# szpiech/garlic

Hardware: AMD Instinct MI355X
Metric: LOD-windows/sec (SNPs x inds / winsize) (higher is better)
Workload: dtype f64

## Files before the change

garlic_amd/csrc/garlic_hip.hip:

```cpp
#include "../../include/garlic_hip.h"
#include "lod_kernels.hpp"
#include "variant_kernels.hpp"
#include "ld_kernels.hpp"
#include "ld_multi_kernel.hpp"
#include "tgls_ring_kernel.hpp"
#include "tgls_wide_kernel.hpp"
#include "tgls_feed_kernel.hpp"
#include "tgls_feed_multi_kernel.hpp"
#include "wlod_strip_kernel.hpp"
#include "wlod_small_kernel.hpp"
#include "coverage_kernel.hpp"
#include "roh_segments_kernel.hpp"
#include "feed_kernel.hpp"
#include "wlod_feed_kernel.hpp"
#include "feed_sort_kernel.hpp"
#include "kde_kernels.hpp"
#include "../host/kde_select.hpp"
#include "bed_kernels.hpp"

#include <algorithm>
#include <chrono>
#include <functional>
#include <memory>
#include <mutex>
// ... 1981 lines not shown
    }
    for (int q = 0; q < 2; q++) {
        size_t blocks = 0;
        for (size_t k = (size_t)q; k < n_slabs; k += 2) blocks = std::max(blocks, (size_t)(slabs[k].b1 - slabs[k].b0));
        const size_t need = blocks * (size_t)rows * WAVE;
        if (need > p->d_slab[q].cap || (!need && p->d_slab[q].cap)) {
            HIP_TRY(hipStreamSynchronize(s));
            p->d_slab[q].release();
            if (need && (rc = p->d_slab[q].reserve(need))) return rc;
        }
    }
    const bool wide = p->gl_wide, wide_host = wide && tgls_terms_on_host(p);
    if (wide) {
        if ((rc = ensure_log10(p->ctx)) || (rc = ensure_dfreq(p)) || (rc = ensure_values16(p))) return rc;
        p->gl_terms_by = p->slab_terms_by = tgls_terms_on_host(p) ? 2 : 1;
    }
    HIP_TRY(hipEventRecord(p->ev_slab_begin, s));
    HIP_TRY(hipStreamWaitEvent(p->slab_stream, p->ev_slab_begin, 0));
    VariantArgs a{p->d_packed.p, nullptr, p->d_tabgl.p, p->d_codes.p, nullptr, nullptr, nullptr, nullptr, nullptr,
                  p->nind_pad, p->nwordrows, 0, 0, 0, (int32_t)p->gl_values.size(), 1, nullptr, 0};
    const size_t terms_lds = sizeof(double) * GL_TERMS_S * 4 * (size_t)a.ncodes;
    if (!wide && terms_lds > LDS_DEFAULT_MAX)
        HIP_TRY(hipFuncSetAttribute((const void *)gl_terms_slab_kernel, hipFuncAttributeMaxDynamicSharedMemorySize, (int)terms_lds));
    const unsigned terms_grid = (unsigned)((p->nloci + GL_TERMS_S - 1) / GL_TERMS_S + (GL_PAD_ROWS + GL_TERMS_S - 1) / GL_TERMS_S);
    for (size_t k = 0; k < n_slabs; k++) {
        const Plan::Slab &sl = slabs[k];
        const int q = (int)(k & 1);
        if (k >= 2) HIP_TRY(hipStreamWaitEvent(p->slab_stream, p->ev_slab_read[q], 0));
        if (wide_host) {
            if ((rc = build_wide_terms_on_host(p, sl.b0, sl.b1, scaled ? p->h_decay.data() : nullptr, p->d_slab[q].p, p->slab_stream, nullptr)))
                return rc;
        } else if (wide)
            launch_wide_terms(p, sl.b0, sl.b1, scaled ? p->d_decay.p : nullptr, p->d_slab[q].p, nullptr, p->slab_stream);
        else
        hipLaunchKernelGGL(gl_terms_slab_kernel, dim3(terms_grid), dim3(256), terms_lds, p->slab_stream, a, p->nloci, rows, sl.b0, sl.b1,
                           scaled ? p->d_decay.p : (const double *)nullptr, p->d_slab[q].p);
        HIP_TRY(hipGetLastError());
        HIP_TRY(hipEventRecord(p->ev_slab_built[q], p->slab_stream));
        HIP_TRY(hipStreamWaitEvent(s, p->ev_slab_built[q], 0));
        if ((rc = chains(k, (const double *)p->d_slab[q].p))) return rc;
        HIP_TRY(hipGetLastError());
        HIP_TRY(hipEventRecord(p->ev_slab_read[q], s));
    }
    return GARLIC_OK;
}

int tgls_workers(const garlic_ctx *ctx, size_t n_items)
{
    int workers = ctx->n_cu;
    if (const char *e = getenv("GARLIC_WORKERS")) workers = std::max(1, atoi(e));
    return std::min<int>(workers, (int)n_items);
}

int launch_tgls_slabs(garlic_panel *p, const LodCall &c, const LodForm &form, const Plan &plan, double *d_out)
{
    hipStream_t s = p->ctx->stream;
    const int64_t rows = GOFF + p->nloci + GPAD_BACK;
    const size_t n_slabs = plan.slabs.size();
    int rc;
    if (n_slabs) {
        if ((rc = p->d_slab_queues.reserve(2 * n_slabs))) return rc;
        HIP_TRY(hipMemsetAsync(p->d_slab_queues.p, 0, 2 * n_slabs * sizeof(int32_t), s));
        if (form.cov_bits) p->cov_written = true;
    }
    return for_each_tgls_slab(p, plan.slabs, form.slab_blocks, [&](size_t k, const double *terms) {
        const Plan::Slab &sl = plan.slabs[k];
        const int workers = tgls_workers(p->ctx, sl.n_items);
        if (form.family == Family::tgls_feed) {
            TglsFeedArgs t{terms, rows, p->d_items.p + sl.item0, p->d_chrs.p, d_out,
                           c.ind_begin, c.ind_count, c.W, (int32_t)sl.n_items, c.thin_step, sl.b0, p->d_slab_queues.p + 2 * k};
            hipLaunchKernelGGL(tgls_feed_kernel, dim3((unsigned)workers), dim3(TGF_THREADS), 0, s, t);
        } else {
            TglsArgs t{terms, rows, p->d_items.p + sl.item0, p->d_chrs.p, d_out,
                       c.ind_begin, c.ind_count, c.W, (int32_t)sl.n_items, sl.b0, p->d_slab_queues.p + 2 * k, p->cov_pending};
            hipLaunchKernelGGL(lod_chain_ring_kernel, dim3((unsigned)workers), dim3(TG_THREADS), 0, s, t);
        }
        return (int)GARLIC_OK;
    });
}

int launch_tgls(garlic_panel *p, const LodCall &c, const LodForm &form, const Plan &plan, int workers, double *d_out)
{
    hipStream_t s = p->ctx->stream;
    const int64_t rows = GOFF + p->nloci + GPAD_BACK;
    if (form.cov_bits && !form.writes_bits) return GARLIC_INTERNAL_NO_BITS;
    p->last_slab_blocks = p->last_n_slabs = 0;
    if (form.slab_blocks && (form.family == Family::tgls_feed || form.family == Family::tgls_ring))
        return launch_tgls_slabs(p, c, form, plan, d_out);
    if (form.family == Family::tgls_feed) {
        TglsFeedArgs t{p->d_glterms.p, rows, p->d_items.p, p->d_chrs.p, d_out,
                       c.ind_begin, c.ind_count, c.W, (int32_t)plan.n_items, c.thin_step, 0, p->d_counter.p};
        hipLaunchKernelGGL(tgls_feed_kernel, dim3((unsigned)workers), dim3(TGF_THREADS), 0, s, t);
        return GARLIC_OK;
    }
    if (form.family == Family::tgls_ring) {
        TglsArgs t{p->d_glterms.p, rows, p->d_items.p, p->d_chrs.p, d_out,
                   c.ind_begin, c.ind_count, c.W, (int32_t)plan.n_items, 0, p->d_counter.p, p->cov_pending};
        if (form.cov_bits) p->cov_written = true;
        hipLaunchKernelGGL(lod_chain_ring_kernel, dim3((unsigned)workers), dim3(TG_THREADS), 0, s, t);
        return GARLIC_OK;
    }
    const VariantArgs a = variant_args(p, c, form, d_out);
    if (form.family == Family::tgls_terms)
        hipLaunchKernelGGL(lod_chain_terms_kernel, dim3((unsigned)plan.n_items), dim3(2 * WAVE), 0, s, a, (int)plan.n_items, rows, p->d_glterms.p);
    else
        hipLaunchKernelGGL(lod_chain_gl_kernel, dim3((unsigned)((plan.n_items + GL_WAVES - 1) / GL_WAVES)), dim3(GL_WAVES * WAVE), 0, s, a,
                           (int)plan.n_items);
    return GARLIC_OK;
}

int launch_generic_wlod(garlic_panel *p, const LodCall &c, const LodForm &form, const Plan &plan, double *d_out)
{
    const int ring = c.W + TILE;
    const size_t lds = sizeof(double) * ((size_t)ring * WAVE + ((c.W + 1) & ~1) + (size_t)WAVE * TPITCH);
    if (lds > 160 * 1024)
        return fail(GARLIC_ERR_INVALID, "wLOD with winsize %d: this build supports 2..240 and 16..4096", c.W);
    HIP_TRY(hipFuncSetAttribute(reinterpret_cast<const void *>(wlod_kernel), hipFuncAttributeMaxDynamicSharedMemorySize, (int)lds));
    hipLaunchKernelGGL(wlod_kernel, dim3((unsigned)plan.n_items), dim3(WAVE), lds, p->ctx->stream, variant_args(p, c, form, d_out), ring);
    return GARLIC_OK;
}

int launch_wlod_feed(garlic_panel *p, const LodCall &c, const LodForm &form, const Plan &plan, double *d_out, const WlodTerms &t,
                     int32_t fb0, int32_t n_fb)
{
    const int nquad = (n_fb + WFD_WAVES - 1) / WFD_WAVES;
    WlodFeedArgs a{p->d_packed.p, form.wlod_gl ? t.terms : p->d_wtab.p, p->d_skew.p + SKEW_FRONT, p->d_valid.p, p->d_chrs.p,
                   p->d_tiles.p, p->d_feed_blocks.p + fb0, d_out, p->nwordrows, GOFF + p->nloci + GPAD_BACK, c.ind_count, c.W, c.thin_step,
                   n_fb, nquad, (uint32_t)((int64_t)plan.n_tiles * nquad), t.blk0};
    if (!a.n_work) return GARLIC_OK;
    if (form.wlod_gl) hipLaunchKernelGGL(wlod_feed_kernel<true>, dim3(a.n_work), dim3(WFD_WAVES * WAVE), 0, p->ctx->stream, a);
    else hipLaunchKernelGGL(wlod_feed_kernel<false>, dim3(a.n_work), dim3(WFD_WAVES * WAVE), 0, p->ctx->stream, a);
    return GARLIC_OK;
}

int launch_wlod_slabs(garlic_panel *p, const LodCall &c, const LodForm &form, const Plan &plan, double *d_out)
{
    return for_each_tgls_slab(p, plan.slabs, form.slab_blocks, [&](size_t k, const double *terms) {
        const Plan::Slab &sl = plan.slabs[k];
        const WlodTerms t = wlod_terms_slab(c, sl, terms);
        if (form.family == Family::wlod_feed) return launch_wlod_feed(p, c, form, plan, d_out, t, sl.fb0, sl.n_fb);
        return launch_wlod(p, c, form, plan, d_out, t);
    }, true);
}

int enqueue_lod(garlic_panel *p, const LodCall &c, const LodForm &form, const Layout &L, Plan &plan, const LodWork *fresh,
                double *d_out, Family family)
{
    garlic_ctx *ctx = p->ctx;
    hipStream_t s = ctx->stream;
    int rc = GARLIC_OK;
    HIP_TRY(hipEventRecord(ctx->ev_begin, s));
    if (fresh && ((rc = p->d_chrs.put(fresh->chrs, s)) || (rc = p->d_items.put(fresh->items, s)) || (rc = p->d_fill.put(fresh->fill, s)) ||
// ... 1160 lines not shown
    return GARLIC_OK;
}
#define LD_COL_FNS(kernel) {kernel<1>, kernel<2>, kernel<3>, kernel<4>, kernel<5>}

static int ld_sum_table(garlic_panel *p, const LdForm &f, std::vector<LdSumChr> &chrs, unsigned *blocks)
{
    int64_t n = 0;
    for (int c = 0; c < p->nchr; c++) {
        const int64_t nstarts = p->chr_off[c + 1] - p->chr_off[c] - f.W + 1;
        if (nstarts < 1) continue;
        chrs.push_back(LdSumChr{p->chr_off[c], nstarts, n});
        n += (nstarts + f.sum_b - 1) / f.sum_b;
    }
    *blocks = (unsigned)n;
    return p->lds.sum_chrs.put(chrs, p->ctx->stream);
}

static int ld_sum_col(garlic_panel *p, const LdForm &f, double *ld, std::vector<LdSumChr> &chrs)
{
    int rc;
    unsigned nwork = 0;
    if ((rc = ld_sum_table(p, f, chrs, &nwork)) || (rc = reserve_skew(p, f.W, false))) return rc;
    if (chrs.empty()) return GARLIC_OK;
    decltype(&ld_sum_col_kernel<1>) const fns[] = LD_COL_FNS(ld_sum_col_kernel);
    return ld_launch_col(p, f, fns, 0, nwork, p->lds.fwd.p, p->lds.sum_chrs.p, (int)chrs.size(), f.W, f.sum_b, ld, p->d_skew.p + SKEW_FRONT);
}

static int ld_sum_two_tables(garlic_panel *p, const LdForm &f, const int32_t *pair, double *ld, std::vector<LdSumChr> &chrs)
{
    int rc;
    hipStream_t s = p->ctx->stream;
    const int32_t W = f.W;
    const size_t n = (size_t)p->nloci * W;
    if ((rc = p->lds.fwd.reserve(n)) || (rc = p->lds.bwd.reserve(n))) return rc;
    for (int c = 0; c < p->nchr; c++) {
        const int64_t lo = p->chr_off[c], hi = p->chr_off[c + 1];
        hipLaunchKernelGGL(ld_hr2_kernel<false>, dim3((unsigned)(hi - lo)), dim3(256), 0, s, pair, p->lds.hf.p, lo, hi, W, p->lds.fwd.p,
                           p->lds.bwd.p);
        if (f.sum == LdSum::plain && hi - lo >= W)
            hipLaunchKernelGGL(ld_sum_kernel, dim3((unsigned)(hi - lo - W + 1)), dim3(256), 0, s, p->lds.fwd.p, p->lds.bwd.p, lo, W, ld);
    }
    if (f.sum == LdSum::plain) return GARLIC_OK;
    unsigned blocks = 0;
    if ((rc = ld_sum_table(p, f, chrs, &blocks))) return rc;
    if (chrs.empty()) return GARLIC_OK;
    const size_t lds = sizeof(double) * 2 * (2 * (size_t)W - 1 + 128 + f.sum_threads);
    (void)hist_mark(p->ctx, false);
    hipLaunchKernelGGL(ld_sum_tiled_kernel, dim3(blocks), dim3(f.sum_threads), lds, s, p->lds.fwd.p, p->lds.bwd.p, p->lds.sum_chrs.p,
                       (int)chrs.size(), W, ld);
    (void)hist_mark(p->ctx, true);
    return GARLIC_OK;
}

static int ld_finish_run(garlic_panel *p, const LdForm &f, const int32_t *loc, const int32_t *pair, double *ld, bool have_table,
                         bool keep_sets)
{
    int rc;
    const bool col = f.sum == LdSum::col;
    if (ld && !col) HIP_TRY(hipMemsetAsync(ld, 0, sizeof(double) * (size_t)p->nloci * f.W, p->ctx->stream));
    if ((ld && col && (rc = ld_zero_short_rows(p, f.W, ld))) || (rc = ld_hf(p, f, loc))) return rc;
    std::vector<LdSumChr> chrs;
    switch (f.sum) {
    case LdSum::flat:
        (void)hist_mark(p->ctx, false);
        hipLaunchKernelGGL(ld_sum_flat_kernel, dim3((unsigned)(((size_t)p->nloci * f.W + 255) / 256)), dim3(256), 0, p->ctx->stream, pair,
                           p->lds.hf.p, p->d_chr_off.p, p->nchr, p->nloci, f.W, ld);
        (void)hist_mark(p->ctx, true);
        break;
    case LdSum::col:
        if (!have_table) rc = ld_build_table(p, f, pair);
        if (!rc) rc = ld_sum_col(p, f, ld, chrs);
        break;
    case LdSum::tiled:
    case LdSum::plain: rc = ld_sum_two_tables(p, f, pair, ld, chrs); break;
    }
    if (rc) return rc;
    HIP_TRY(hipGetLastError());
    return install_ld(p, f.W, ld, col, keep_sets);
}

static int ld_copy_out(double *dst, const double *src, size_t n, int32_t where)
{
    HIP_TRY(hipMemcpy(dst, src, sizeof(double) * n, where == GARLIC_HOST ? hipMemcpyDeviceToHost : hipMemcpyDeviceToDevice));
    return GARLIC_OK;
}

static int ld_finish_to(garlic_panel *p, const LdForm &f, const int32_t *loc, const int32_t *pair, bool have_table, double *ld_out,
                        bool host_out, bool keep_sets)
{
    int rc;
    const size_t n = (size_t)p->nloci * f.W;
    double *ld = host_out ? nullptr : ld_out;
    if (!ld && (ld_out || f.sum != LdSum::col)) {
        if ((rc = p->lds.ld.reserve(n))) return rc;
        ld = p->lds.ld.p;
    }
    if ((rc = ld_finish_run(p, f, loc, pair, ld, have_table, keep_sets))) return rc;
    return ld_out && ld != ld_out ? ld_copy_out(ld_out, ld, n, GARLIC_HOST) : GARLIC_OK;
}

int garlic_ld_finish(garlic_panel *p, int32_t winsize, int32_t phased, const int32_t *locus_counts,
                     const int32_t *pair_counts, double *ld_out, int32_t where)
{
    int rc;
    if ((rc = ld_check(p, winsize, phased))) return rc;
    if (!locus_counts || !pair_counts) return fail(GARLIC_ERR_INVALID, "count buffers are required");
    hipStream_t s = p->ctx->stream;
    if (where == GARLIC_HOST) {
        DevBuf<int32_t> &d_loc = p->lds.loc, &d_pair = p->lds.pair;
        const size_t npair = (size_t)p->nloci * winsize * 2;
        if ((rc = d_loc.reserve((size_t)p->nloci * 2)) || (rc = d_pair.reserve(npair))) return rc;
        HIP_TRY(hipMemcpyAsync(d_loc.p, locus_counts, sizeof(int32_t) * p->nloci * 2, hipMemcpyHostToDevice, s));
        HIP_TRY(hipMemcpyAsync(d_pair.p, pair_counts, sizeof(int32_t) * npair, hipMemcpyHostToDevice, s));
        locus_counts = d_loc.p; pair_counts = d_pair.p;
    }
    const LdForm f = ld_form(p, winsize, phased);
    ld_note_form(p, f, false);
    return ld_finish_to(p, f, locus_counts, pair_counts, false, ld_out, where == GARLIC_HOST, false);
}

static int ld_compute(garlic_panel *p, const LdForm &f, const std::vector<uint64_t> &sub, double *ld_out, bool host_out, bool keep_sets)
{
    int rc;
    DevBuf<int32_t> &d_loc = p->lds.loc, &d_pair = p->lds.pair;
    ld_note_form(p, f, f.fusable);
    if ((rc = d_loc.reserve((size_t)p->nloci * 2)) || (rc = d_pair.reserve(f.fusable ? 2 : (size_t)p->nloci * f.W * 2))) return rc;
    if ((rc = ld_counts_run(p, f, sub, d_loc.p, d_pair.p, f.fusable))) return rc;
    return ld_finish_to(p, f, d_loc.p, d_pair.p, f.fusable, ld_out, host_out, keep_sets);
}

int garlic_panel_compute_ld(garlic_panel *p, int32_t winsize, int32_t phased, const int32_t *sub_idx,
                            int32_t n_sub, double *ld_out, int32_t where)
{
    int rc;
    if ((rc = ld_check(p, winsize, phased))) return rc;
    std::vector<uint64_t> sub;
    if ((rc = ld_sub_bitmap(p, sub_idx, n_sub, sub))) return rc;
    return ld_compute(p, ld_form(p, winsize, phased), sub, ld_out, where != GARLIC_DEVICE, false);
}

struct LdMultiPlan {
    std::vector<int32_t> uniq;
    std::vector<std::vector<int32_t>> groups;
    size_t n_shared = 0;
    int32_t wtab = 0;
};
// ... 1107 lines not shown
            a_w0 = d_w0.p;
        }
        hipLaunchKernelGGL(roh_segments_from_mask_kernel, grid, dim3(256), 0, s, d_mask.p, bm.d_bchrs.p, d_brk.p, bm.d_wbase.p, p->nchr, p->nind, T,
                           d_segs.p, (long long)cap, d_count.p, a_w0);
        e = hipGetLastError();
        if (e == hipSuccess) e = hipMemcpyAsync(&found, d_count.p, sizeof found, hipMemcpyDeviceToHost, s);
        if (e == hipSuccess) e = hipStreamSynchronize(s);
        if (e != hipSuccess) return fail(GARLIC_ERR_HIP, "roh segments: %s", hipGetErrorString(e));
    }
    if (sink.n_out) *sink.n_out = (int64_t)found;
    if ((int64_t)found <= cap && found > 0) {
        e = hipMemcpyAsync(sink.segs, d_segs.p, sizeof(garlic_roh_segment) * found, hipMemcpyDeviceToHost, s);
        if (e == hipSuccess) e = hipStreamSynchronize(s);
        if (e != hipSuccess) return fail(GARLIC_ERR_HIP, "roh segments: %s", hipGetErrorString(e));
        std::sort(sink.segs, sink.segs + found, [](const garlic_roh_segment &x, const garlic_roh_segment &y) {
            return x.ind != y.ind ? x.ind < y.ind : x.chr != y.chr ? x.chr < y.chr : x.start < y.start;
        });
    }
    return GARLIC_OK;
}

static int coverage_unfused(garlic_panel *p, const CovSink &c)
{
    hipStream_t s = p->ctx->stream;
    const Layout L = make_layout(p, 32, p->nind);
    int rc;
    if ((rc = p->d_out.reserve(p->ctx, (size_t)L.total))) return rc;
    if (c.weighted) rc = garlic_wlod_windows(p, c.W, c.error, c.max_gap, c.use_gl, c.M, c.mu, 0, p->nind, 32, p->d_out.p, GARLIC_DEVICE);
    else rc = garlic_lod_windows(p, c.W, c.error, c.max_gap, c.use_gl, 0, p->nind, 32, p->d_out.p, GARLIC_DEVICE);
    if (rc) return rc;
    if (!c.segments) return garlic_roh_coverage(p, p->d_out.p, 32, p->nind, c.W, c.cutoff, c.inwin, c.inwin_pitch_align, c.where);
    const std::vector<ChrDev> schrs = chr_table(p, L);
    BitMatrix bm;
    DevBuf<ChrDev> d_schrs;
    if ((rc = bm.make(p, 1)) || (rc = d_schrs.put(schrs, s))) return rc;
    if (bm.word_base[(size_t)p->nchr] > 0)
        hipLaunchKernelGGL(roh_bits_from_scores_kernel, dim3((unsigned)((bm.word_base[(size_t)p->nchr] + 255) / 256), (unsigned)p->nind),
                           dim3(256), 0, s, p->d_out.p, d_schrs.p, bm.d_bchrs.p, bm.d_wbase.p, p->nchr, c.W, c.cutoff, bm.d_bits.p);
    const hipError_t e = hipStreamSynchronize(s);
    if (e != hipSuccess) return fail(GARLIC_ERR_HIP, "roh segments: %s", hipGetErrorString(e));
    return segments_from_bits(p, bm, c);
}

static int coverage_from_score_kernels(garlic_panel *p, const CovSink &c)
{
    hipStream_t s = p->ctx->stream;
    const Layout Lo = make_layout(p, c.inwin_pitch_align, p->nind);
    const std::vector<ChrDev> ochrs = chr_table(p, Lo);
    BitMatrix bm;
    DevBuf<ChrDev> d_ochrs;
    DevBuf<int16_t> d_cov;
    int16_t *dst;
    int rc;
    if ((rc = bm.make(p, 1)) || (rc = d_ochrs.put(ochrs, s)) || (rc = counts_target(c.inwin, c.where, Lo, d_cov, &dst))) return rc;
    hipError_t e = bm.zero(s);
    if (e == hipSuccess) e = hipStreamSynchronize(s);
    if (e != hipSuccess) return fail(GARLIC_ERR_HIP, "coverage: %s", hipGetErrorString(e));
    p->cov_pending = CovBits{bm.d_bits.p, bm.d_bchrs.p, c.cutoff};
    p->cov_written = false;
    double *bits_as_out = reinterpret_cast<double *>(bm.d_bits.p);
    if (c.weighted) rc = garlic_wlod_windows(p, c.W, c.error, c.max_gap, c.use_gl, c.M, c.mu, 0, p->nind, 32, bits_as_out, GARLIC_DEVICE);
    else rc = garlic_lod_windows(p, c.W, c.error, c.max_gap, 1, 0, p->nind, 32, bits_as_out, GARLIC_DEVICE);
    const bool written = c.weighted || p->cov_written;
    p->cov_pending = CovBits{nullptr, nullptr, 0.0};
    if (rc == GARLIC_INTERNAL_NO_BITS) return coverage_unfused(p, c);
    if (rc) return rc;
    if (!written) return coverage_unfused(p, c);
    if (c.segments) return segments_from_bits(p, bm, c);
    launch_counts_from_bits(p, bm, c, Lo, d_ochrs.p, dst);
    return finish_counts(p, c.inwin, c.where, Lo, dst, nullptr);
}

static int coverage_lod_bits(garlic_panel *p, const CovSink &c)
{
    garlic_ctx *ctx = p->ctx;
    hipStream_t s = ctx->stream;
    const int32_t W = c.W;
    const size_t nchr = (size_t)p->nchr;
    std::vector<Run> runs;
    std::vector<FillItem> fill;
    int64_t n_valid = 0;
    plan_runs(p, W, runs, fill, n_valid);
    std::vector<int32_t> col0(runs.size(), 0);
    std::vector<FeedItem> items;
    build_feed_items(runs, longest_first(runs), nullptr, (p->nind + WAVE - 1) / WAVE, col0, items);
    const Layout Lo = make_layout(p, c.inwin_pitch_align, p->nind);
    const std::vector<ChrDev> chrs = chr_table(p, Lo);
    BitMatrix bm;
    DevBuf<FeedItem> d_items;
    DevBuf<ChrDev> d_chrs;
    DevBuf<int32_t> d_counter, d_cnt;
    DevBuf<int16_t> d_cov;
    int16_t *dst;
    int rc;
    if ((rc = d_items.put(items, s)) || (rc = d_chrs.put(chrs, s)) || (rc = d_counter.reserve(4)) || (rc = counts_target(c.inwin, c.where, Lo, d_cov, &dst)))
        return rc;
    hipError_t e = hipMemsetAsync(d_counter.p, 0, 4 * sizeof(int32_t), s);
    if (e != hipSuccess) return fail(GARLIC_ERR_HIP, "coverage: %s", hipGetErrorString(e));
    const bool vec_ok = cov_vec_ok(p, Lo, dst);
    if ((rc = bm.make(p, 8))) return rc;
    (void)hist_mark(ctx, false);
    if ((e = bm.zero(s)) != hipSuccess) return fail(GARLIC_ERR_HIP, "coverage: %s", hipGetErrorString(e));
    const bool overlap = !items.empty() && !c.segments && getenv("GARLIC_COVERAGE_OVERLAP");
    int64_t n_cnt_items = 0;
    if (overlap) {
        std::vector<int32_t> h(4 * nchr + 2, 0);
        int32_t *need = h.data() + nchr + 1, *corder = need + nchr, *cbase = corder + nchr;
// ... 543 lines not shown
```

garlic_amd/csrc/tgls_ring_kernel.hpp:

```cpp
#pragma once
#include "variant_kernels.hpp"

namespace garlic {

#ifndef GARLIC_TG_RING
#define GARLIC_TG_RING 240
#endif
#ifndef GARLIC_TG_DEPTH
#define GARLIC_TG_DEPTH 3
#endif
#ifndef GARLIC_TG_TILE_ROWS
#define GARLIC_TG_TILE_ROWS WAVE
#endif
constexpr int TG_RING = GARLIC_TG_RING;
constexpr int TG_GROUP = 8;
constexpr int TG_DEPTH = GARLIC_TG_DEPTH;
constexpr int TG_THREADS = 4 * WAVE;
constexpr int TG_SINGLE_MAX_W = TG_RING - 32 - 4 * TG_GROUP * 2;

struct TglsArgs {
    const double *terms;
    int64_t term_rows;
    const ChainItem *items;
    const ChrDev *chrs;
    double *out;
    int32_t ind_begin, ind_count, winsize, n_items;
    int32_t blk0;
    int32_t *next_item;
    CovBits cov;
};

__device__ __forceinline__ int tg_flag_read(const int *flag)
{
    int v;
    const uint32_t a = (uint32_t)(uintptr_t)(const __attribute__((address_space(3))) int *)flag;
    asm volatile("ds_read_b32 %0, %1\n\ts_waitcnt lgkmcnt(0)" : "=v"(v) : "v"(a) : "memory");
    return __builtin_amdgcn_readfirstlane(v);
}
__device__ __forceinline__ void tg_flag_write(int *flag, int v)
{
    const uint32_t a = (uint32_t)(uintptr_t)(__attribute__((address_space(3))) int *)flag;
    asm volatile("ds_write_b32 %0, %1\n\ts_waitcnt lgkmcnt(0)" ::"v"(a), "v"(v) : "memory");
}

__device__ __forceinline__ void tg_loader(const double *src, int n_req, int piece_step, int w, int ring_rows,
                                          uint32_t ring_lds, const int *tiles_done, int *landed, int lane)
{
    const uint32_t lane16 = (uint32_t)lane * 16u;
    const uint32_t ring_bytes = (uint32_t)ring_rows * 512u;
    const uint32_t step_bytes = (uint32_t)piece_step * 1024u;
    uint32_t slot_off = (piece_step == 2 ? (uint32_t)w : 0u) * 1024u;
    const double *gp = src + (piece_step == 2 ? w : 0) * 128;
    int issued = 0, landed_n = 0;
    int inflight = 0;
    while (issued < n_req) {
        const int n = min(TG_GROUP, n_req - issued);
        const int g_last = piece_step * (issued + n - 1) + (piece_step == 2 ? w : 0);
        const int need_done = (2 * g_last + 2 - ring_rows + 31) / 32;
        if (need_done > 0 && tg_flag_read(tiles_done) < need_done) {
            asm volatile("s_waitcnt vmcnt(0)" ::: "memory");
            if (landed_n != issued) tg_flag_write(landed, issued);
            landed_n = issued;
            inflight = 0;
            while (tg_flag_read(tiles_done) < need_done) __builtin_amdgcn_s_sleep(2);
        }
#pragma unroll
        for (int q = 0; q < TG_GROUP; q++) {
            if (q < n) {
                asm volatile("s_mov_b32 m0, %0\n\ts_nop 0\n\tglobal_load_lds_dwordx4 %1, %2"
                             :: "s"(ring_lds + slot_off), "v"(lane16), "s"(gp) : "memory");
                slot_off += step_bytes;
                if (slot_off >= ring_bytes) slot_off -= ring_bytes;
                gp += piece_step * 128;
            }
        }
        issued += n;
        if (n < TG_GROUP) break;
        if (++inflight == TG_DEPTH) {
            asm volatile("s_waitcnt vmcnt(%0)" ::"n"(TG_GROUP * (TG_DEPTH - 1)) : "memory");
            landed_n += TG_GROUP;
            tg_flag_write(landed, landed_n);
            inflight--;
        }
    }
    asm volatile("s_waitcnt vmcnt(0)" ::: "memory");
    tg_flag_write(landed, n_req);
}

__global__ void __launch_bounds__(TG_THREADS)
lod_chain_ring_kernel(TglsArgs p)
{
    __shared__ __attribute__((aligned(1024))) double ring[TG_RING * WAVE];
    __shared__ __attribute__((aligned(16))) double tiles[2][GARLIC_TG_TILE_ROWS * TPITCH];
    __shared__ int flags[8];
    const int lane = threadIdx.x & (WAVE - 1);
    const int wave = __builtin_amdgcn_readfirstlane(threadIdx.x >> 6);
    const uint32_t ring_lds = (uint32_t)(uintptr_t)(__attribute__((address_space(3))) double *)ring;
    for (;;) {
        if (threadIdx.x == 0) {
            flags[4] = atomicAdd(p.next_item, 1);
            flags[0] = 0; flags[1] = 0; flags[2] = 0; flags[3] = 0;
        }
        __syncthreads();
        const int item_idx = __builtin_amdgcn_readfirstlane(flags[4]);
        if (item_idx >= p.n_items) {
            if (threadIdx.x == 0) {
                __threadfence();
                if (atomicAdd(p.next_item + 1, 1) == (int)gridDim.x - 1) {
                    p.next_item[0] = 0;
                    p.next_item[1] = 0;
                }
            }
            return;
        }
        const ChainItem it = p.items[item_idx];
        const ChrDev c = p.chrs[it.chr];
        const int W = p.winsize, a = it.a, b = it.b;
        const int first = a & ~(TILE - 1);
        const int ntiles = (b - first) / TILE + 1;
        const bool single = W <= TG_SINGLE_MAX_W;
        const int ring_rows = single ? TG_RING : TG_RING / 2;
        const int64_t col0 = (int64_t)p.ind_begin + it.ind0;
        const int64_t Gbase = c.loc_base + GOFF;
        const double *blk = p.terms + (((col0 >> 6) - p.blk0) * p.term_rows) * WAVE;
        const double *trail = blk + (Gbase + first - 1) * WAVE;
        const double *lead = blk + (Gbase + first + W - 1) * WAVE;

        if (wave < 2) {
            if (single) {
                const int n_rows = TILE * ntiles + W;
                const int n_pieces = (n_rows + 1) / 2;
                const int mine = (n_pieces - wave + 1) / 2;
                tg_loader(trail, mine, 2, wave, ring_rows, ring_lds, &flags[0], &flags[2 + wave], lane);
            } else {
                const int n_pieces = TILE * ntiles / 2;
                tg_loader(wave == 0 ? lead : trail, n_pieces, 1, 0, ring_rows,
                          ring_lds + (wave == 0 ? 0u : (uint32_t)ring_rows * 512u), &flags[0], &flags[2 + wave], lane);
            }
        } else if (wave == 3 && p.cov.bits) {
        } else if (wave == 3) {
            const int rows_valid = min(WAVE, p.ind_count - it.ind0);
            double *out_row0 = p.out + c.out_base + (int64_t)it.ind0 * c.out_pitch;
            for (int k = 0; k < ntiles; k++) {
                while (LDS_FLAG_GET(flags[0]) <= k) __builtin_amdgcn_s_sleep(1);
                lds_acquire();
                variant_store(tiles[k & 1], first + k * TILE, a, b, lane, rows_valid, out_row0 + first + k * TILE, c.out_pitch);
                lds_release();
                if (lane == 0) LDS_FLAG_SET(flags[1], k + 1);
            }
        } else {
            const double *tcol = blk + lane;
            double acc = 0.0;
            for (int l0 = a; l0 < a + W - 1; l0 += 32) {
                double t[32];
#pragma unroll
                for (int q = 0; q < 32; q++) t[q] = tcol[(Gbase + min(l0 + q, a + W - 2)) * WAVE];
#pragma unroll
                for (int q = 0; q < 32; q++) acc += (l0 + q < a + W - 1) ? t[q] : 0.0;
            }
            int so = 0, si = single ? W % ring_rows : 0;
            const int base_out = single ? 0 : ring_rows * WAVE;
            uint32_t *bits_row = nullptr;
            if (p.cov.bits) {
                const ChrDev bc = p.cov.bchrs[it.chr];
                bits_row = p.cov.bits + bc.out_base + (int64_t)(it.ind0 + lane) * bc.out_pitch;
            }
            for (int k = 0; k < ntiles; k++) {
#ifndef GARLIC_TG_ABL_NOWAIT
                if (single) {
                    const int pieces = (TILE * (k + 1) + W + 1) / 2;
                    const int need0 = (pieces + 1) / 2, need1 = pieces / 2;
                    while (LDS_FLAG_GET(flags[2]) < need0 || LDS_FLAG_GET(flags[3]) < need1) __builtin_amdgcn_s_sleep(1);
                } else {
                    const int need = TILE * (k + 1) / 2;
                    while (LDS_FLAG_GET(flags[2]) < need || LDS_FLAG_GET(flags[3]) < need) __builtin_amdgcn_s_sleep(1);
                }
#endif
                const bool bits_mode = p.cov.bits != nullptr;
                if (!bits_mode)
                    while (LDS_FLAG_GET(flags[1]) + 2 <= k) __builtin_amdgcn_s_sleep(1);
                lds_acquire();
                double *tile = tiles[k & 1];
                const int s0 = first + k * TILE;
                const bool edge = (s0 <= a) || (s0 + TILE - 1 > b);
                double t_in[TILE], t_out[TILE];
                if (si + TILE <= ring_rows && so + TILE <= ring_rows) {
                    const double *pi = ring + si * WAVE + lane, *po = ring + base_out + so * WAVE + lane;
#pragma unroll
                    for (int j = 0; j < TILE; j++) {
#ifdef GARLIC_TG_ABL_NOREADS
                        t_in[j] = (double)(j + k);
                        t_out[j] = (double)(j - k);
#else
                        t_in[j] = pi[j * WAVE];
                        t_out[j] = po[j * WAVE];
#endif
                    }
                    si = (si + TILE == ring_rows) ? 0 : si + TILE;
                    so = (so + TILE == ring_rows) ? 0 : so + TILE;
                } else {
#pragma unroll
                    for (int j = 0; j < TILE; j++) {
                        t_in[j] = ring[si * WAVE + lane];
                        t_out[j] = ring[base_out + so * WAVE + lane];
                        si = (si + 1 == ring_rows) ? 0 : si + 1;
                        so = (so + 1 == ring_rows) ? 0 : so + 1;
                    }
                }
                if (bits_mode) {
                    uint32_t m = 0;
                    const double cutoff = p.cov.cutoff;
                    if (edge) {
#pragma unroll
                        for (int j = 0; j < TILE; j++) {
                            const int s = s0 + j;
                            const bool in = (s >= a && s <= b);
                            const double ti = in ? t_in[j] : 0.0;
                            const double to = (in && s > a) ? t_out[j] : 0.0;
                            acc = (acc - to) + ti;
                            m |= (in && acc >= cutoff) ? (1u << j) : 0u;
                        }
                    } else {
#ifdef GARLIC_TG_ABL_NOCOMPUTE
                        asm volatile("" :: "v"(t_in[0]), "v"(t_out[0]), "v"(t_in[TILE - 1]), "v"(t_out[TILE - 1]));
#else
#pragma unroll
                        for (int j = 0; j < TILE; j++) {
                            acc = (acc - t_out[j]) + t_in[j];
                            m |= (acc >= cutoff) ? (1u << j) : 0u;
                        }
#endif
                    }
                    if (it.ind0 + lane < p.ind_count) {
                        uint32_t *w = bits_row + (s0 >> 5);
                        if (edge) { if (m) atomicOr(w, m); }
                        else *w = m;
                    }
                } else if (edge) {
#pragma unroll
                    for (int j = 0; j < TILE; j++) {
                        const int s = s0 + j;
                        const bool in = (s >= a && s <= b);
                        const double ti = in ? t_in[j] : 0.0;
                        const double to = (in && s > a) ? t_out[j] : 0.0;
                        acc = (acc - to) + ti;
                        tile[lane * TPITCH + j] = acc;
                    }
                } else {
#pragma unroll
                    for (int j = 0; j < TILE; j++) {
                        acc = (acc - t_out[j]) + t_in[j];
                        tile[lane * TPITCH + j] = acc;
                    }
                }
                lds_release();
                if (lane == 0) LDS_FLAG_SET(flags[0], k + 1);
            }
        }
        __syncthreads();
    }
}

}
```

garlic_amd/csrc/ld_kernels.hpp:

```cpp
#pragma once
#include "lod_kernels.hpp"
#include "tgls_math.hpp"
#include "variant_kernels.hpp"

namespace garlic {

__device__ __forceinline__ double x86_nan_if_nan(double v)
{
    return v != v ? f64_from_bits(X86_DEFAULT_NAN) : v;
}

__device__ __forceinline__ uint32_t ld_writelane(uint32_t v, int lane, uint32_t old)
{
    asm("v_writelane_b32 %0, %1, %2" : "+v"(old) : "s"(v), "n"(lane));
    return old;
}

template <bool PHASED>
__global__ void __launch_bounds__(256)
ld_planes_kernel(const uint32_t *__restrict__ packed, int64_t nwordrows, int nblk,
                 const uint64_t *__restrict__ submask, int64_t nloci, uint64_t *__restrict__ planeM,
                 uint64_t *__restrict__ planeH, uint64_t *__restrict__ planeO, int32_t *__restrict__ counts)
{
    __shared__ int32_t red[4][16][2];
// ... 304 lines not shown
                    if (PHASED) {
                        const ulonglong2 c1 = *reinterpret_cast<const ulonglong2 *>(cp + 2);
                        tot[r] += 2 * __popcll(a0.x & c0.x);
                        hab[r] += 2 * __popcll(a0.y & c0.y) + __popcll(a1.x & c0.y) + __popcll(a0.y & c1.x) +
                                  __popcll(a1.x & c1.x & ~(a1.y ^ c1.y));
                    } else {
                        tot[r] += __popcll(a0.x & c0.x);
                        hab[r] += __popcll(a0.y & c0.y);
                    }
                }
            }
        }
        if (mine) {
            int32_t *row = pair + (i0 + i) * (int64_t)W * 2;
            if (d0 == 1) *reinterpret_cast<int2 *>(row) = make_int2(0, 0);
#pragma unroll
            for (int r = 0; r < LD_LANE_DC; r++)
                if (d0 + r < W) *reinterpret_cast<int2 *>(row + (d0 + r) * 2) = make_int2(tot[r], hab[r]);
        }
    }
}

constexpr int LD_SMALL_MAX_W = 16;

template <bool PHASED>
__global__ void __launch_bounds__(256)
ld_pair_flat_kernel(const uint64_t *__restrict__ planeM, const uint64_t *__restrict__ planeH,
                    const uint64_t *__restrict__ planeO, const uint64_t *__restrict__ planeF, int nblk, int64_t nloci,
                    const int64_t *__restrict__ chr_off, int nchr, int W, int32_t *__restrict__ pair)
{
    const int64_t e = (int64_t)blockIdx.x * blockDim.x + threadIdx.x;
    if (e >= nloci * W) return;
    const int64_t i = e / W;
    const int d = (int)(e - i * W);
    const int64_t j = i + d;
    int32_t tot = 0, hab = 0;
    if (d > 0 && j < nloci && j < chr_off[find_chr(chr_off, nchr, i) + 1]) {
        for (int blk = 0; blk < nblk; blk++) {
            const int64_t base = (int64_t)blk * nloci;
            if (PHASED) {
                const uint64_t ti = planeH[base + i], tj = planeH[base + j], oi = planeO[base + i], oj = planeO[base + j];
                tot += 2 * __popcll(planeM[base + i] & planeM[base + j]);
                hab += 2 * __popcll(ti & tj) + __popcll(oi & tj) + __popcll(ti & oj) +
                       __popcll(oi & oj & ~(planeF[base + i] ^ planeF[base + j]));
            } else {
                tot += __popcll(planeM[base + i] & planeM[base + j]);
                hab += __popcll(planeH[base + i] & planeH[base + j]);
            }
        }
    }
    *reinterpret_cast<int2 *>(pair + e * 2) = make_int2(tot, hab);
}

__global__ void __launch_bounds__(256)
ld_sum_flat_kernel(const int32_t *__restrict__ pair, const double *__restrict__ hf, const int64_t *__restrict__ chr_off,
                   int nchr, int64_t nloci, int W, double *__restrict__ ld)
{
    const int64_t e = (int64_t)blockIdx.x * blockDim.x + threadIdx.x;
    if (e >= nloci * W) return;
    const int64_t s = e / W;
    const int k = (int)(e - s * W);
    if (s + W > chr_off[find_chr(chr_off, nchr, s) + 1]) return;
    const int64_t t = s + k;
    const double HT = hf[t];
    double acc = 0.0;
    for (int64_t i = s; i < s + W; i++) {
        double term = 1.0;
        if (i < t) {
            const int2 c = *reinterpret_cast<const int2 *>(pair + (i * W + (t - i)) * 2);
            term = hr2_from_counts(hf[i], HT, c.y, c.x);
        } else if (i > t) {
            const int2 c = *reinterpret_cast<const int2 *>(pair + (t * W + (i - t)) * 2);
            term = hr2_from_counts(hf[i], HT, c.y, c.x);
        }
        acc += term;
    }
    ld[e] = x86_nan_if_nan(acc);
}

#ifndef GARLIC_LD_HR2_T
#define GARLIC_LD_HR2_T 32
#endif
constexpr int LD_HR2_T = GARLIC_LD_HR2_T;
__global__ void __launch_bounds__(256)
ld_hr2_tile_kernel(const int32_t *__restrict__ pair, const double *__restrict__ hf, int64_t lo, int64_t hi,
                   int W, double *__restrict__ C)
{
    extern __shared__ double hr2_lds[];
    const int pitch = W + (W & 1);
    double *hfl = hr2_lds, *tile = hr2_lds + LD_HR2_T + W;
    const int64_t i0 = lo + (int64_t)blockIdx.x * LD_HR2_T;
    for (int e = threadIdx.x; e < LD_HR2_T + W - 1; e += blockDim.x) hfl[e] = (i0 + e < hi) ? hf[i0 + e] : 0.0;
    __syncthreads();
    for (int e = threadIdx.x; e < LD_HR2_T * W; e += blockDim.x) {
        const int ii = e / W, d = e - ii * W;
        const int64_t i = i0 + ii, j = i + d;
        if (j >= hi) continue;
        if (d == 0) { C[i * 2 * W + W - 1] = 1.0; continue; }
        const int2 cnt = *reinterpret_cast<const int2 *>(pair + (i * W + d) * 2);
        const double HA = hfl[ii], HB = hfl[ii + d];
        double f = 0.0, b = 0.0;
        if (HA > 0 && HA < 1 && HB > 0 && HB < 1) {
            double HAB = (double)cnt.y;
            HAB /= (double)cnt.x;
            const double H = HAB - HA * HB, HH = H * H;
            const double vf = HH / (HA * (1 - HA) * HB * (1 - HB));
            const double vb = HH / (HB * (1 - HB) * HA * (1 - HA));
            f = (vf > 1) ? 1.0 : x86_nan_if_nan(vf);
            b = (vb > 1) ? 1.0 : x86_nan_if_nan(vb);
        }
        C[i * 2 * W + W - 1 + d] = f;
        tile[ii * pitch + d] = b;
    }
    __syncthreads();
    const int nrows = LD_HR2_T + W - 2;
    for (int e = threadIdx.x; e < nrows * LD_HR2_T; e += blockDim.x) {
        const int jj = e / LD_HR2_T, ii = e - jj * LD_HR2_T;
        const int d = jj + 1 - ii;
        const int64_t j = i0 + 1 + jj;
        if (d < 1 || d >= W || j >= hi) continue;
        C[j * 2 * W + W - 1 - d] = tile[ii * pitch + d];
    }
}

__global__ void __launch_bounds__(256)
ld_sum_kernel(const double *__restrict__ fwd, const double *__restrict__ bwd, int64_t lo, int W,
              double *__restrict__ ld)
{
    const int64_t s = lo + blockIdx.x;
    for (int k = threadIdx.x; k < W; k += blockDim.x) {
// ... 475 lines not shown
```

Baseline: 7.344 billion.

## Add specialized bits-mode ring kernel with three waves, deeper ring and vector bit stores

Splits the ring chain kernel into a templated body and adds a coverage-bits variant. The variant drops the writer wave and tile buffers, uses a larger LDS ring and deeper loader prefetch, and reads the landed flags uniformly. It builds each mask with a compare-and-carry sequence, gathers eight words per lane and writes them as two 16-byte stores when aligned, falling back to the old per-word path otherwise. Unweighted coverage bit matrices are now allocated with a wider alignment so the vector stores apply. The trade-offs are inline asm with a reversed bit order that must match the old layout, plus added code and LDS pressure.

```diff
diff --git a/garlic_amd/csrc/garlic_hip.hip b/garlic_amd/csrc/garlic_hip.hip
--- a/garlic_amd/csrc/garlic_hip.hip
+++ b/garlic_amd/csrc/garlic_hip.hip
@@ -2057,6 +2057,12 @@
     return std::min<int>(workers, (int)n_items);
 }
 
+static void launch_ring_chain(const TglsArgs &t, int workers, hipStream_t s)
+{
+    if (t.cov.bits) hipLaunchKernelGGL(lod_chain_ring_bits_kernel, dim3((unsigned)workers), dim3(TG_BITS_THREADS), 0, s, t);
+    else hipLaunchKernelGGL(lod_chain_ring_kernel, dim3((unsigned)workers), dim3(TG_THREADS), 0, s, t);
+}
+
 int launch_tgls_slabs(garlic_panel *p, const LodCall &c, const LodForm &form, const Plan &plan, double *d_out)
 {
     hipStream_t s = p->ctx->stream;
@@ -2078,7 +2084,7 @@
         } else {
             TglsArgs t{terms, rows, p->d_items.p + sl.item0, p->d_chrs.p, d_out,
                        c.ind_begin, c.ind_count, c.W, (int32_t)sl.n_items, sl.b0, p->d_slab_queues.p + 2 * k, p->cov_pending};
-            hipLaunchKernelGGL(lod_chain_ring_kernel, dim3((unsigned)workers), dim3(TG_THREADS), 0, s, t);
+            launch_ring_chain(t, workers, s);
         }
         return (int)GARLIC_OK;
     });
@@ -2102,7 +2108,7 @@
         TglsArgs t{p->d_glterms.p, rows, p->d_items.p, p->d_chrs.p, d_out,
                    c.ind_begin, c.ind_count, c.W, (int32_t)plan.n_items, 0, p->d_counter.p, p->cov_pending};
         if (form.cov_bits) p->cov_written = true;
-        hipLaunchKernelGGL(lod_chain_ring_kernel, dim3((unsigned)workers), dim3(TG_THREADS), 0, s, t);
+        launch_ring_chain(t, workers, s);
         return GARLIC_OK;
     }
     const VariantArgs a = variant_args(p, c, form, d_out);
@@ -4622,7 +4628,7 @@
     DevBuf<int16_t> d_cov;
     int16_t *dst;
     int rc;
-    if ((rc = bm.make(p, 1)) || (rc = d_ochrs.put(ochrs, s)) || (rc = counts_target(c.inwin, c.where, Lo, d_cov, &dst))) return rc;
+    if ((rc = bm.make(p, c.weighted ? 1 : 8)) || (rc = d_ochrs.put(ochrs, s)) || (rc = counts_target(c.inwin, c.where, Lo, d_cov, &dst))) return rc;
     hipError_t e = bm.zero(s);
     if (e == hipSuccess) e = hipStreamSynchronize(s);
     if (e != hipSuccess) return fail(GARLIC_ERR_HIP, "coverage: %s", hipGetErrorString(e));
diff --git a/garlic_amd/csrc/tgls_ring_kernel.hpp b/garlic_amd/csrc/tgls_ring_kernel.hpp
--- a/garlic_amd/csrc/tgls_ring_kernel.hpp
+++ b/garlic_amd/csrc/tgls_ring_kernel.hpp
@@ -16,6 +16,20 @@
 constexpr int TG_GROUP = 8;
 constexpr int TG_DEPTH = GARLIC_TG_DEPTH;
 constexpr int TG_THREADS = 4 * WAVE;
+#ifndef GARLIC_TG_BITS_WAVES
+#define GARLIC_TG_BITS_WAVES 3
+#endif
+constexpr int TG_BITS_THREADS = GARLIC_TG_BITS_WAVES * WAVE;
+#ifndef GARLIC_TG_BITS_RING
+#define GARLIC_TG_BITS_RING 312
+#endif
+#ifndef GARLIC_TG_BITS_DEPTH
+#define GARLIC_TG_BITS_DEPTH 5
+#endif
+constexpr int TG_BITS_RING = GARLIC_TG_BITS_RING;
+constexpr int TG_BITS_DEPTH = GARLIC_TG_BITS_DEPTH;
+static_assert(TG_BITS_RING % 8 == 0 && TG_BITS_RING >= TG_RING && TG_BITS_RING * 512 + 64 <= 160 * 1024, "bits ring: whole requests, within a CU's LDS");
+static_assert(TG_GROUP * TG_BITS_DEPTH <= 63 && TG_GROUP * TG_DEPTH <= 63, "a loader's requests are counted in vmcnt");
 constexpr int TG_SINGLE_MAX_W = TG_RING - 32 - 4 * TG_GROUP * 2;
 
 struct TglsArgs {
@@ -43,6 +57,7 @@
     asm volatile("ds_write_b32 %0, %1\n\ts_waitcnt lgkmcnt(0)" ::"v"(a), "v"(v) : "memory");
 }
 
+template <int DEPTH = TG_DEPTH>
 __device__ __forceinline__ void tg_loader(const double *src, int n_req, int piece_step, int w, int ring_rows,
                                           uint32_t ring_lds, const int *tiles_done, int *landed, int lane)
 {
@@ -76,8 +91,8 @@
         }
         issued += n;
         if (n < TG_GROUP) break;
-        if (++inflight == TG_DEPTH) {
-            asm volatile("s_waitcnt vmcnt(%0)" ::"n"(TG_GROUP * (TG_DEPTH - 1)) : "memory");
+        if (++inflight == DEPTH) {
+            asm volatile("s_waitcnt vmcnt(%0)" ::"n"(TG_GROUP * (DEPTH - 1)) : "memory");
             landed_n += TG_GROUP;
             tg_flag_write(landed, landed_n);
             inflight--;
@@ -87,12 +102,9 @@
     tg_flag_write(landed, n_req);
 }
 
-__global__ void __launch_bounds__(TG_THREADS)
-lod_chain_ring_kernel(TglsArgs p)
-{
-    __shared__ __attribute__((aligned(1024))) double ring[TG_RING * WAVE];
-    __shared__ __attribute__((aligned(16))) double tiles[2][GARLIC_TG_TILE_ROWS * TPITCH];
-    __shared__ int flags[8];
+template <bool BITS, int RING, int DEPTH>
+__device__ __forceinline__ void tg_ring_items(const TglsArgs &p, double *ring, double (*tiles)[GARLIC_TG_TILE_ROWS * TPITCH], int *flags)
+{
     const int lane = threadIdx.x & (WAVE - 1);
     const int wave = __builtin_amdgcn_readfirstlane(threadIdx.x >> 6);
     const uint32_t ring_lds = (uint32_t)(uintptr_t)(__attribute__((address_space(3))) double *)ring;
@@ -119,7 +131,7 @@
         const int first = a & ~(TILE - 1);
         const int ntiles = (b - first) / TILE + 1;
         const bool single = W <= TG_SINGLE_MAX_W;
-        const int ring_rows = single ? TG_RING : TG_RING / 2;
+        const int ring_rows = single ? RING : RING / 2;
         const int64_t col0 = (int64_t)p.ind_begin + it.ind0;
         const int64_t Gbase = c.loc_base + GOFF;
         const double *blk = p.terms + (((col0 >> 6) - p.blk0) * p.term_rows) * WAVE;
@@ -131,13 +143,13 @@
                 const int n_rows = TILE * ntiles + W;
                 const int n_pieces = (n_rows + 1) / 2;
                 const int mine = (n_pieces - wave + 1) / 2;
-                tg_loader(trail, mine, 2, wave, ring_rows, ring_lds, &flags[0], &flags[2 + wave], lane);
+                tg_loader<DEPTH>(trail, mine, 2, wave, ring_rows, ring_lds, &flags[0], &flags[2 + wave], lane);
             } else {
                 const int n_pieces = TILE * ntiles / 2;
-                tg_loader(wave == 0 ? lead : trail, n_pieces, 1, 0, ring_rows,
+                tg_loader<DEPTH>(wave == 0 ? lead : trail, n_pieces, 1, 0, ring_rows,
                           ring_lds + (wave == 0 ? 0u : (uint32_t)ring_rows * 512u), &flags[0], &flags[2 + wave], lane);
             }
-        } else if (wave == 3 && p.cov.bits) {
+        } else if (BITS && wave == 3) {
         } else if (wave == 3) {
             const int rows_valid = min(WAVE, p.ind_count - it.ind0);
             double *out_row0 = p.out + c.out_base + (int64_t)it.ind0 * c.out_pitch;
@@ -161,26 +173,42 @@
             int so = 0, si = single ? W % ring_rows : 0;
             const int base_out = single ? 0 : ring_rows * WAVE;
             uint32_t *bits_row = nullptr;
-            if (p.cov.bits) {
+            int kp0 = 0, kp1 = 0;
+            const int w0 = first >> 5;
+            if (BITS) {
                 const ChrDev bc = p.cov.bchrs[it.chr];
                 bits_row = p.cov.bits + bc.out_base + (int64_t)(it.ind0 + lane) * bc.out_pitch;
-            }
+                const int k_last = (first + TILE * ntiles - 1 > b) ? ntiles - 2 : ntiles - 1;
+                kp0 = ((w0 + 8) & ~7) - w0;
+                kp1 = kp0 + (max(0, k_last + 1 - kp0) & ~7);
+                if (((bc.out_base | bc.out_pitch) & 7) != 0 || ((uintptr_t)p.cov.bits & 31) != 0) kp1 = kp0;
+            }
+            uint32_t pc[8] = {0, 0, 0, 0, 0, 0, 0, 0};
+            int have0 = 0, have1 = 0;
             for (int k = 0; k < ntiles; k++) {
 #ifndef GARLIC_TG_ABL_NOWAIT
+                int need0, need1;
                 if (single) {
                     const int pieces = (TILE * (k + 1) + W + 1) / 2;
-                    const int need0 = (pieces + 1) / 2, need1 = pieces / 2;
+                    need0 = (pieces + 1) / 2, need1 = pieces / 2;
+                } else {
+                    need0 = need1 = TILE * (k + 1) / 2;
+                }
+                if (BITS) {
+                    while (have0 < need0 || have1 < need1) {
+                        have0 = __builtin_amdgcn_readfirstlane(LDS_FLAG_GET(flags[2]));
+                        have1 = __builtin_amdgcn_readfirstlane(LDS_FLAG_GET(flags[3]));
+                        if (have0 < need0 || have1 < need1) __builtin_amdgcn_s_sleep(1);
+                    }
+                } else {
                     while (LDS_FLAG_GET(flags[2]) < need0 || LDS_FLAG_GET(flags[3]) < need1) __builtin_amdgcn_s_sleep(1);
-                } else {
-                    const int need = TILE * (k + 1) / 2;
-                    while (LDS_FLAG_GET(flags[2]) < need || LDS_FLAG_GET(flags[3]) < need) __builtin_amdgcn_s_sleep(1);
-                }
-#endif
-                const bool bits_mode = p.cov.bits != nullptr;
+                }
+#endif
+                constexpr bool bits_mode = BITS;
                 if (!bits_mode)
                     while (LDS_FLAG_GET(flags[1]) + 2 <= k) __builtin_amdgcn_s_sleep(1);
                 lds_acquire();
-                double *tile = tiles[k & 1];
+                double *tile = BITS ? nullptr : tiles[k & 1];
                 const int s0 = first + k * TILE;
                 const bool edge = (s0 <= a) || (s0 + TILE - 1 > b);
                 double t_in[TILE], t_out[TILE];
@@ -227,11 +255,22 @@
 #pragma unroll
                         for (int j = 0; j < TILE; j++) {
                             acc = (acc - t_out[j]) + t_in[j];
-                            m |= (acc >= cutoff) ? (1u << j) : 0u;
+                            asm("v_cmp_le_f64 vcc, %2, %1\n\tv_addc_co_u32 %0, vcc, %0, %0, vcc" : "+v"(m) : "v"(acc), "s"(cutoff) : "vcc");
                         }
-#endif
-                    }
-                    if (it.ind0 + lane < p.ind_count) {
+                        m = __builtin_bitreverse32(m);
+#endif
+                    }
+                    const bool row = it.ind0 + lane < p.ind_count;
+                    if (k >= kp0 && k < kp1) {
+                        const int q = (w0 + k) & 7;
+#pragma unroll
+                        for (int i = 0; i < 8; i++) pc[i] = (q == i) ? m : pc[i];
+                        if (q == 7 && row) {
+                            uint4 *w = reinterpret_cast<uint4 *>(bits_row + (w0 + k - 7));
+                            w[0] = make_uint4(pc[0], pc[1], pc[2], pc[3]);
+                            w[1] = make_uint4(pc[4], pc[5], pc[6], pc[7]);
+                        }
+                    } else if (row) {
                         uint32_t *w = bits_row + (s0 >> 5);
                         if (edge) { if (m) atomicOr(w, m); }
                         else *w = m;
@@ -261,4 +300,21 @@
     }
 }
 
-}
+__global__ void __launch_bounds__(TG_THREADS)
+lod_chain_ring_kernel(TglsArgs p)
+{
+    __shared__ __attribute__((aligned(1024))) double ring[TG_RING * WAVE];
+    __shared__ __attribute__((aligned(16))) double tiles[2][GARLIC_TG_TILE_ROWS * TPITCH];
+    __shared__ int flags[8];
+    tg_ring_items<false, TG_RING, TG_DEPTH>(p, ring, tiles, flags);
+}
+
+__global__ void __launch_bounds__(TG_BITS_THREADS)
+lod_chain_ring_bits_kernel(TglsArgs p)
+{
+    __shared__ __attribute__((aligned(1024))) double ring[TG_BITS_RING * WAVE];
+    __shared__ int flags[8];
+    tg_ring_items<true, TG_BITS_RING, TG_BITS_DEPTH>(p, ring, nullptr, flags);
+}
+
+}
```

Result: slower. 7.256 billion (-1.2%).

## Replace flat LD sum with LDS-tiled narrow-window kernel emitting weights directly

Applied to the files above, without the earlier changes.

The per-element flat LD summation kernel, which re-read pair counts and recomputed hr2 terms W times per output, is replaced by a block-tiled kernel. It stages hf and the forward/backward hr2 matrix for a tile of SNPs in shared memory, sums the diagonals from there, and writes the ld sums plus the skewed reciprocal weights directly. The flat path is now treated like the column path, so the memset and the separate weight install step are skipped. LDS use grows as O((T+W)·W), which limits this to small windows and may reduce occupancy.

```diff
diff --git a/garlic_amd/csrc/garlic_hip.hip b/garlic_amd/csrc/garlic_hip.hip
--- a/garlic_amd/csrc/garlic_hip.hip
+++ b/garlic_amd/csrc/garlic_hip.hip
@@ -3369,21 +3369,32 @@
     return GARLIC_OK;
 }
 
+static int ld_sum_narrow(garlic_panel *p, const LdForm &f, const int32_t *pair, double *ld, std::vector<LdPairChr> &tiles)
+{
+    int rc;
+    unsigned blocks = 0;
+    if ((rc = ld_pair_table(p, LD_NARROW_T, tiles, &blocks)) || (rc = reserve_skew(p, f.W, false))) return rc;
+    if (blocks == 0) return GARLIC_OK;
+    (void)hist_mark(p->ctx, false);
+    hipLaunchKernelGGL(ld_sum_narrow_kernel, dim3(blocks), dim3(LD_NARROW_THREADS), ld_narrow_lds_bytes(f.W), p->ctx->stream, pair,
+                       p->lds.hf.p, p->lds.pair_chrs.p, p->nchr, f.W, ld, p->d_skew.p + SKEW_FRONT);
+    (void)hist_mark(p->ctx, true);
+    return GARLIC_OK;
+}
+
+static bool ld_sum_writes_weights(const LdForm &f) { return f.sum == LdSum::col || f.sum == LdSum::flat; }
+
 static int ld_finish_run(garlic_panel *p, const LdForm &f, const int32_t *loc, const int32_t *pair, double *ld, bool have_table,
                          bool keep_sets)
 {
     int rc;
     const bool col = f.sum == LdSum::col;
-    if (ld && !col) HIP_TRY(hipMemsetAsync(ld, 0, sizeof(double) * (size_t)p->nloci * f.W, p->ctx->stream));
+    if (ld && !ld_sum_writes_weights(f)) HIP_TRY(hipMemsetAsync(ld, 0, sizeof(double) * (size_t)p->nloci * f.W, p->ctx->stream));
     if ((ld && col && (rc = ld_zero_short_rows(p, f.W, ld))) || (rc = ld_hf(p, f, loc))) return rc;
     std::vector<LdSumChr> chrs;
+    std::vector<LdPairChr> tiles;
     switch (f.sum) {
-    case LdSum::flat:
-        (void)hist_mark(p->ctx, false);
-        hipLaunchKernelGGL(ld_sum_flat_kernel, dim3((unsigned)(((size_t)p->nloci * f.W + 255) / 256)), dim3(256), 0, p->ctx->stream, pair,
-                           p->lds.hf.p, p->d_chr_off.p, p->nchr, p->nloci, f.W, ld);
-        (void)hist_mark(p->ctx, true);
-        break;
+    case LdSum::flat: rc = ld_sum_narrow(p, f, pair, ld, tiles); break;
     case LdSum::col:
         if (!have_table) rc = ld_build_table(p, f, pair);
         if (!rc) rc = ld_sum_col(p, f, ld, chrs);
@@ -3393,7 +3404,7 @@
     }
     if (rc) return rc;
     HIP_TRY(hipGetLastError());
-    return install_ld(p, f.W, ld, col, keep_sets);
+    return install_ld(p, f.W, ld, ld_sum_writes_weights(f), keep_sets);
 }
 
 static int ld_copy_out(double *dst, const double *src, size_t n, int32_t where)
@@ -3408,7 +3419,7 @@
     int rc;
     const size_t n = (size_t)p->nloci * f.W;
     double *ld = host_out ? nullptr : ld_out;
-    if (!ld && (ld_out || f.sum != LdSum::col)) {
+    if (!ld && (ld_out || !ld_sum_writes_weights(f))) {
         if ((rc = p->lds.ld.reserve(n))) return rc;
         ld = p->lds.ld.p;
     }
diff --git a/garlic_amd/csrc/ld_kernels.hpp b/garlic_amd/csrc/ld_kernels.hpp
--- a/garlic_amd/csrc/ld_kernels.hpp
+++ b/garlic_amd/csrc/ld_kernels.hpp
@@ -380,30 +380,101 @@
     *reinterpret_cast<int2 *>(pair + e * 2) = make_int2(tot, hab);
 }
 
-__global__ void __launch_bounds__(256)
-ld_sum_flat_kernel(const int32_t *__restrict__ pair, const double *__restrict__ hf, const int64_t *__restrict__ chr_off,
-                   int nchr, int64_t nloci, int W, double *__restrict__ ld)
-{
-    const int64_t e = (int64_t)blockIdx.x * blockDim.x + threadIdx.x;
-    if (e >= nloci * W) return;
-    const int64_t s = e / W;
-    const int k = (int)(e - s * W);
-    if (s + W > chr_off[find_chr(chr_off, nchr, s) + 1]) return;
-    const int64_t t = s + k;
-    const double HT = hf[t];
-    double acc = 0.0;
-    for (int64_t i = s; i < s + W; i++) {
-        double term = 1.0;
-        if (i < t) {
-            const int2 c = *reinterpret_cast<const int2 *>(pair + (i * W + (t - i)) * 2);
-            term = hr2_from_counts(hf[i], HT, c.y, c.x);
-        } else if (i > t) {
-            const int2 c = *reinterpret_cast<const int2 *>(pair + (t * W + (i - t)) * 2);
-            term = hr2_from_counts(hf[i], HT, c.y, c.x);
-        }
-        acc += term;
-    }
-    ld[e] = x86_nan_if_nan(acc);
+constexpr int LD_NARROW_T = 128;
+constexpr int LD_NARROW_THREADS = 256;
+constexpr int LD_NARROW_ITEMS = LD_NARROW_T * LD_SMALL_MAX_W / LD_NARROW_THREADS;
+__host__ __device__ constexpr size_t ld_narrow_lds_bytes(int W)
+{
+    return sizeof(double) * (size_t)(LD_NARROW_T + W - 1) * (size_t)(2 * W);
+}
+__global__ void __launch_bounds__(LD_NARROW_THREADS)
+ld_sum_narrow_kernel(const int32_t *__restrict__ pair, const double *__restrict__ hf, const LdPairChr *__restrict__ chrs,
+                     int nchr, int W, double *__restrict__ ld, double *__restrict__ D)
+{
+    static_assert((LD_NARROW_T & (LD_NARROW_T - 1)) == 0 && LD_NARROW_THREADS % LD_NARROW_T == 0, "lanes along s");
+    extern __shared__ double ldn_lds[];
+    constexpr int T = LD_NARROW_T, NT = LD_NARROW_THREADS;
+    const int span = T + W - 1, P = 2 * W - 1, PR = W | 1;
+    double *hfl = ldn_lds, *C = ldn_lds + span, *R = C;
+    int c = 0;
+    while (c + 1 < nchr && (int64_t)blockIdx.x >= chrs[c + 1].block0) c++;
+    const int64_t lo = chrs[c].lo, hi = chrs[c].hi;
+    const int64_t s0 = lo + ((int64_t)blockIdx.x - chrs[c].block0) * T;
+    const int nsnp = (int)min<int64_t>(span, hi - s0);
+    const int tid = threadIdx.x;
+    for (int e = tid; e < span; e += NT) hfl[e] = e < nsnp ? hf[s0 + e] : 0.0;
+    __syncthreads();
+    const int qstep = NT / W, rstep = NT - qstep * W;
+    {
+        const int32_t *prow = pair + s0 * W * 2;
+        int ii = tid / W, d = tid - ii * W;
+        for (int e = tid; e < span * W; e += NT) {
+            if (ii + d < nsnp) {
+                if (d == 0) {
+                    C[ii * P + W - 1] = 1.0;
+                } else {
+                    const int2 cnt = *reinterpret_cast<const int2 *>(prow + (size_t)e * 2);
+                    const double HA = hfl[ii], HB = hfl[ii + d];
+                    double f = 0.0, b = 0.0;
+                    if (HA > 0 && HA < 1 && HB > 0 && HB < 1) {
+                        double HAB = (double)cnt.y;
+                        HAB /= (double)cnt.x;
+                        const double H = HAB - HA * HB, HH = H * H;
+                        const double vf = HH / (HA * (1 - HA) * HB * (1 - HB));
+                        const double vb = HH / (HB * (1 - HB) * HA * (1 - HA));
+                        f = (vf > 1) ? 1.0 : x86_nan_if_nan(vf);
+                        b = (vb > 1) ? 1.0 : x86_nan_if_nan(vb);
+                    }
+                    C[ii * P + W - 1 + d] = f;
+                    C[(ii + d) * P + W - 1 - d] = b;
+                }
+            }
+            ii += qstep;
+            d += rstep;
+            if (d >= W) { d -= W; ii++; }
+        }
+    }
+    __syncthreads();
+    double acc[LD_NARROW_ITEMS];
+#pragma unroll
+    for (int u = 0; u < LD_NARROW_ITEMS; u++) {
+        const int item = tid + u * NT, s = item & (T - 1), k = item / T;
+        acc[u] = 0.0;
+        if (k < W && s + W <= nsnp) {
+            const double *cp = C + s * P + k + W - 1;
+            double a = 0.0;
+            for (int m = 0; m < W; m++) a += cp[m * (P - 1)];
+            acc[u] = x86_nan_if_nan(a);
+        }
+    }
+    __syncthreads();
+#pragma unroll
+    for (int u = 0; u < LD_NARROW_ITEMS; u++) {
+        const int item = tid + u * NT, s = item & (T - 1), k = item / T;
+        if (k < W) R[s * PR + k] = acc[u];
+    }
+    __syncthreads();
+    if (ld) {
+        const int nrow = (int)min<int64_t>(T, hi - s0);
+        int s = tid / W, k = tid - s * W;
+        for (int e = tid; e < nrow * W; e += NT) {
+            ld[s0 * W + e] = R[s * PR + k];
+            s += qstep;
+            k += rstep;
+            if (k >= W) { k -= W; s++; }
+        }
+    }
+    {
+        int l = tid / W, j = tid - l * W;
+        for (int e = tid; e < nsnp * W; e += NT) {
+            const int s = l - j;
+            if (s >= 0 && s < T) D[s0 * W + e] = reciprocal_x86(R[s * PR + j]);
+            else if (s < 0 && s0 == lo) D[s0 * W + e] = 0.0;
+            l += qstep;
+            j += rstep;
+            if (j >= W) { j -= W; l++; }
+        }
+    }
 }
 
 #ifndef GARLIC_LD_HR2_T
```

Result: slower. 7.359 billion before, 7.276 billion after (-1.1%).
